# wdmwhh/MRefSR

Hardware: NVIDIA B200
Metric: x4 SR images/sec through the reference-alignment hot path (match + DCNv2 + fusion), 5 refs @160^2 HR (higher is better)
Workload: dtype f32 I/O (matcher: split-bf16 x3 operands on tcgen05, fp32 accumulate, diagonal form; dcn: tf32 operands, fp32 accumulate; fusion: fp32)

## Files before the change

include/mrefsr_b200.h:

```cpp
#ifndef MREFSR_B200_H_
#define MREFSR_B200_H_

#include <stddef.h>
#include <stdint.h>

#ifdef __cplusplus
extern "C" {
#endif

#define MREFSR_ABI_VERSION 1

#if defined(__GNUC__)
#define MREFSR_API __attribute__((visibility("default")))
#else
#define MREFSR_API
#endif

MREFSR_API int mrefsr_abi_version(void);
MREFSR_API const char* mrefsr_last_error(void);
MREFSR_API int mrefsr_sm_count(void);

enum {
    MREFSR_MATCH_AUTO = 0,
    MREFSR_MATCH_TC_BF16X3 = 1,
// ... 16 lines not shown
                                 void* stream);

MREFSR_API int mrefsr_pre_offsets(const int64_t* max_idx, int n, int h, int w, float* out_s1, float* out_s2, float* out_s4,
                       void* stream);

enum {
    MREFSR_DCN_AUTO = 0,
    MREFSR_DCN_FP32 = 1,
    MREFSR_DCN_TF32 = 2,
    MREFSR_DCN_TF32X3 = 3,
};
MREFSR_API size_t mrefsr_dcn_workspace_bytes(int B, int C, int H, int W, int Co, int kh, int kw, int stride_h, int stride_w,
                                  int pad_h, int pad_w, int dil_h, int dil_w, int group, int deformable_group,
                                  int mode, int backward);
MREFSR_API int mrefsr_dcn_tile_plan(int B, int Ho, int Wo, int* meta, int* coords, size_t max_rows);
MREFSR_API int mrefsr_modulated_deform_conv_forward(const float* input, const float* weight, const float* bias,
                                         const float* offset, const float* mask, float* output, int B, int C, int H,
                                         int W, int Co, int kh, int kw, int stride_h, int stride_w, int pad_h,
                                         int pad_w, int dil_h, int dil_w, int group, int deformable_group,
                                         int with_bias, int mode, void* workspace, size_t workspace_bytes,
                                         void* stream);
MREFSR_API int mrefsr_modulated_deform_conv_backward(const float* input, const float* weight, const float* offset,
                                          const float* mask, const float* grad_output, float* grad_input,
                                          float* grad_weight, float* grad_bias, float* grad_offset, float* grad_mask,
                                          int B, int C, int H, int W, int Co, int kh, int kw, int stride_h,
                                          int stride_w, int pad_h, int pad_w, int dil_h, int dil_w, int group,
                                          int deformable_group, int with_bias, int mode, void* workspace,
                                          size_t workspace_bytes, void* stream);

MREFSR_API int mrefsr_dynagg_offsets(const float* conv_out, const float* pre_offset, float* offset, float* mask,
// ... 118 lines not shown
```

mrefsr_b200/_lib.py:

```python
import ctypes
import os
import threading

import torch

_HERE = os.path.dirname(os.path.abspath(__file__))
LIB_PATH = os.environ.get('MREFSR_LIB') or os.path.join(_HERE, 'lib', 'libmrefsr_b200.so')

c_int, c_size_t, c_void_p = ctypes.c_int, ctypes.c_size_t, ctypes.c_void_p

_I = c_int
_P = c_void_p
SIGNATURES = {
    'mrefsr_abi_version': (c_int, []),
    'mrefsr_last_error': (ctypes.c_char_p, []),
    'mrefsr_sm_count': (c_int, []),
    'mrefsr_match_workspace_bytes': (c_size_t, [_I] * 8),
    'mrefsr_match_plan': (c_int, [_I] * 9 + [_P]),
    'mrefsr_feature_match_batched': (c_int, [_P, _P] + [_I] * 15 + [_P, _P, _P, c_size_t, _P]),
    'mrefsr_pre_offsets': (c_int, [_P, _I, _I, _I, _P, _P, _P, _P]),
    'mrefsr_dcn_workspace_bytes': (c_size_t, [_I] * 17),
    'mrefsr_dcn_tile_plan': (c_int, [_I, _I, _I, _P, _P, c_size_t]),
    'mrefsr_modulated_deform_conv_forward': (c_int, [_P] * 6 + [_I] * 17 + [_P, c_size_t, _P]),
    'mrefsr_modulated_deform_conv_backward': (c_int, [_P] * 10 + [_I] * 17 + [_P, c_size_t, _P]),
    'mrefsr_gemm_tf32_nt': (c_int, [_P, _I, ctypes.c_longlong, _P, _I, ctypes.c_longlong, _P, _I, ctypes.c_longlong,
                                    _I, _I, _I, _I, _I, _I, _P]),
    'mrefsr_gemm_tf32x3_nt': (c_int, [_P, _P, _I, ctypes.c_longlong, _P, _P, _I, ctypes.c_longlong, _P, _I,
                                      ctypes.c_longlong, _I, _I, _I, _I, _I, _I, _P]),
    'mrefsr_dcn_pack_weights': (c_int, [_P, _P, _I, _I, _I, _P]),
    'mrefsr_dcn_pack_weights_x3': (c_int, [_P, _P, _I, _I, _I, _P]),
    'mrefsr_dynagg_dcn_forward': (c_int, [_P] * 5 + [_I] + [_P] + [_I] * 7 + [_P, c_size_t, _P]),
    'mrefsr_dynagg_dcn_forward_multi': (c_int, [_P] * 5 + [_I] + [_P] + [_I] * 12 + [ctypes.c_float, _P, c_size_t, _P]),
    'mrefsr_dynagg_dcn_forward_slabs': (c_int, [_P] * 5 + [_I] + [_P] + [_I] * 13 + [ctypes.c_float, _P, c_size_t, _P]),
    'mrefsr_dynagg_dcn_forward_ex': (c_int, [_P] * 5 + [_I] + [_P] + [_I] * 8 + [ctypes.c_float, _P, c_size_t, _P]),
    'mrefsr_dynagg_dcn_backward': (c_int, [_P] * 4 + [_I] + [_P] * 5 + [_I] * 9 + [_P, c_size_t, _P]),
    'mrefsr_dynagg_offsets': (c_int, [_P] * 5 + [_I] * 5 + [_P]),
    'mrefsr_dynagg_offsets_backward': (c_int, [_P] * 4 + [_I] * 5 + [_P]),
# ... 101 lines not shown
```

mrefsr_b200/csrc/dcn.cu:

```cuda
#include <type_traits>

#include "common.cuh"
#include "dcn_tc.cuh"
#include "../../include/mrefsr_b200.h"

namespace mrefsr {

constexpr int DT = 64;
constexpr int DK = 16;

__global__ void __launch_bounds__(256)
dcn_fwd_simt_kernel(const float* __restrict__ x, const float* __restrict__ offset, const float* __restrict__ mask,
                    const float* __restrict__ weight, const float* __restrict__ bias, float* __restrict__ out,
                    const DcnShape s) {
    __shared__ float As[DK][DT + 4];
    __shared__ float Bs[DK][DT + 4];
    const int K = s.kh * s.kw, P = s.Ho * s.Wo, cpg = s.C / s.G, opg = s.Co / s.G, cdg = s.C / s.DG;
    const int oct = cdiv_d(opg, DT);
    const int b = blockIdx.z, gi = blockIdx.y / oct, ot = blockIdx.y % oct;
    const int p0 = blockIdx.x * DT, oc0 = ot * DT;
    const int t = threadIdx.x;
    const int lpos = t & 63, lkq = (t >> 6) * 4;
    const int ty = t >> 4, tx = t & 15;
    const int p = p0 + lpos;
// ... 956 lines not shown
    return 0;
}

}

using namespace mrefsr;

extern "C" {

int mrefsr_dcn_tile_plan(int B, int Ho, int Wo, int* meta, int* coords, size_t max_rows) {
    MREFSR_CHECK(B > 0 && Ho > 0 && Wo > 0 && meta, ERR_BAD_ARG, "tile plan: bad arguments");
    MREFSR_CHECK((long long)B * Ho * Wo < (1ll << 31) - 256, ERR_BAD_ARG, "tile plan: too many positions");
    return dcn_tc_tile_plan(B, Ho, Wo, meta, coords, max_rows);
}

size_t mrefsr_dcn_workspace_bytes(int B, int C, int H, int W, int Co, int kh, int kw, int stride_h, int stride_w,
                                  int pad_h, int pad_w, int dil_h, int dil_w, int group, int deformable_group, int mode,
                                  int backward) {
    DcnShape s;
    if (dcn_make_shape(&s, B, C, H, W, Co, kh, kw, stride_h, stride_w, pad_h, pad_w, dil_h, dil_w, group,
                       deformable_group))
        return 0;
    if (backward) {
        const bool x3 = mode == MREFSR_DCN_TF32X3;
        const size_t buf = align_up((size_t)bwd_chunk(s, x3) * C * kh * kw * s.Ho * s.Wo * 4, 1024);
        const size_t got = align_up((size_t)B * Co * s.Ho * s.Wo * 4, 1024), gwt = align_up((size_t)Co * C * kh * kw * 4, 1024);
        return 2 * buf + align_up((size_t)B * C * H * W * 4, 1024) + 2 * got + 2 * gwt +
               align_up((size_t)BWD_MAX_SPLITS * Co * C * kh * kw * 4, 1024) + (x3 ? buf + 2 * got + gwt : 0) + 1024;
    }
    return dcn_tc_workspace_bytes(s, mode) + 1024;
// ... 279 lines not shown
```

mrefsr_b200/csrc/dcn_common.cuh:

```cuda
#pragma once
#include "common.cuh"

namespace mrefsr {

struct DcnShape {
    int B, C, H, W, Co, kh, kw, sh, sw, ph, pw, dh, dw, G, DG, Ho, Wo;
};

__host__ __device__ __forceinline__ int cdiv_d(int a, int b) { return (a + b - 1) / b; }

struct PlaneSrc {};
struct DynAggSrc {
    const long long* max_idx;
    int flow_scale, hp, wp, x_nhwc;
};

#ifdef __CUDACC__
__device__ __forceinline__ float dcn_sample(const float* __restrict__ plane, int H, int W, float y, float x) {
    if (!(y > -1.f && x > -1.f && y < (float)H && x < (float)W)) return 0.f;
    const int y0 = (int)floorf(y), x0 = (int)floorf(x);
    const int y1 = y0 + 1, x1 = x0 + 1;
    const float ly = y - (float)y0, lx = x - (float)x0, hy = 1.f - ly, hx = 1.f - lx;
    const float a = (y0 >= 0 && x0 >= 0) ? __ldg(plane + y0 * W + x0) : 0.f;
    const float b = (y0 >= 0 && x1 <= W - 1) ? __ldg(plane + y0 * W + x1) : 0.f;
// ... 19 lines not shown
int dcn_pack_weights(const float* w, float* wt, int Co, int C, int K, cudaStream_t st, bool x3 = false);

struct DcnOutputs {
    float* ptr[8];
    int n, group, stride, offset;
    int slab_rows;
};

bool dcn_tc_eligible(const DcnShape& s);
size_t dcn_tc_workspace_bytes(const DcnShape& s, int mode);
int dcn_forward_tc_impl(const float* x, const float* w, const float* bias, const float* off, const float* mask,
                        const long long* max_idx, int flow_scale, float* out, const DcnShape& s, void* workspace,
                        size_t workspace_bytes, cudaStream_t st, int layout_flags, float out_slope,
                        const DcnOutputs* multi);
int dcn_tc_tile_plan(int B, int Ho, int Wo, int* meta, int* coords, size_t max_rows);
int dcn_forward_tc(const float* x, const float* w, const float* bias, const float* off, const float* mask, float* out,
                   const DcnShape& s, void* workspace, size_t workspace_bytes, cudaStream_t st, bool x3);

}
```

mrefsr_b200/csrc/dcn_tc.cu:

```cuda
#include <stdlib.h>
#include "dcn_tc.cuh"
#include "../../include/mrefsr_b200.h"

namespace mrefsr {


template <bool ROUND,
          bool SPLIT = false>
__global__ void __launch_bounds__(256)
nchw_to_nhwc_kernel(const float* __restrict__ src, float* __restrict__ dst, int C, int HW, float* __restrict__ dst_lo) {
    __shared__ float tile[128][33];
    const int b = blockIdx.z, p0 = blockIdx.x * 32, c0 = blockIdx.y * 128;
    const int lane = threadIdx.x & 31, warp = threadIdx.x >> 5;
    const float* s = src + (size_t)b * C * HW;
    float* d = dst + (size_t)b * C * HW;
    const int p = p0 + lane;
#pragma unroll
    for (int i = 0; i < 16; ++i) {
        const int cl = warp + 8 * i, c = c0 + cl;
        const float v = (c < C && p < HW) ? __ldcs(s + (size_t)c * HW + p) : 0.f;
        tile[cl][lane] = (ROUND && !SPLIT) ? to_tf32(v) : v;
    }
    __syncthreads();
#pragma unroll
// ... 23 lines not shown
}

__global__ void dcn_weight_repack_x3_kernel(const float* __restrict__ w, float* __restrict__ wt, int Co, int C, int K) {
    const int total = Co * C * K;
    for (int i = blockIdx.x * blockDim.x + threadIdx.x; i < total; i += gridDim.x * blockDim.x) {
        const int c = i % C, tap = (i / C) % K, co = i / (C * K);
        const float v = __ldg(w + ((size_t)co * C + c) * K + tap), hi = to_tf32(v);
        float* o = wt + ((size_t)co * K + tap) * 2 * C + (c / TBK_X3) * 2 * TBK_X3 + c % TBK_X3;
        o[0] = hi;
        o[TBK_X3] = to_tf32(v - hi);
    }
}


__device__ __forceinline__ void dcn_epilogue_tile(const DcnTcParams& prm, const float* __restrict__ bias,
                                                  uint32_t tmem_base, uint64_t* tempty_bar, int tile, int buf, int warp,
                                                  int lane, int half_lo, int half_hi) {
    const int Co = prm.s.Co, P = prm.P;
#pragma unroll 1
    for (int half = half_lo; half < half_hi; ++half) {
        int b = 0, oy = 0, ox = 0;
        const bool ok = dcn_row_coords(prm, tile, half * 128 + warp * 32 + lane, b, oy, ox);
        const int p = ok ? oy * prm.s.Wo + ox : 0;
        if (!ok) b = 0;
        const int bd = prm.dst_group ? (b / prm.dst_group) * prm.dst_stride + prm.dst_offset + b % prm.dst_group : b;
        int k_lo = 0, k_hi = prm.n_outs, Pd = P;
        size_t o_off = prm.out_nhwc ? ((size_t)bd * P + p) * Co : (size_t)bd * Co * P + p;
        if (prm.dst_slab_rows) {
            k_lo = oy / prm.dst_slab_rows;
            k_hi = k_lo + 1;
            Pd = prm.dst_slab_rows * prm.s.Wo;
            o_off = (size_t)bd * Co * Pd + (size_t)(oy - k_lo * prm.dst_slab_rows) * prm.s.Wo + ox;
        }
        const uint32_t taddr = tmem_base + ((uint32_t)(warp * 32) << 16) + buf * 2 * Co + half * Co;
#pragma unroll 1
        for (int c0 = 0; c0 < Co; c0 += 8) {
            uint32_t v[8];
            tmem_ld_32x8(taddr + c0, v);
            tmem_ld_wait();
#ifdef MREFSR_DCN_DEBUG
            if (prm.dbg & 16) continue;
#endif
            if (ok) {
                float f[8];
#pragma unroll
                for (int e = 0; e < 8; ++e) {
                    f[e] = __uint_as_float(v[e]) + (bias ? __ldg(bias + c0 + e) : 0.f);
                    f[e] = f[e] > 0.f ? f[e] : f[e] * prm.out_slope;
                }
#pragma unroll 1
                for (int k = k_lo; k < k_hi; ++k) {
                    float* o = prm.outs[k] + o_off;
                    if (prm.out_nhwc) {
                        *reinterpret_cast<float4*>(o + c0) = make_float4(f[0], f[1], f[2], f[3]);
                        *reinterpret_cast<float4*>(o + c0 + 4) = make_float4(f[4], f[5], f[6], f[7]);
                    } else {
#pragma unroll
                        for (int e = 0; e < 8; ++e) o[(size_t)(c0 + e) * Pd] = f[e];
                    }
                }
            }
        }
    }
    tc_fence_before();
    __syncwarp();
    if (lane == 0) mbar_arrive(tempty_bar);
}

template <bool X3>
__device__ __forceinline__ void dcn_mma_issuer(const DcnTcParams& prm, uint8_t* smem, uint64_t* full, uint64_t* empty,
                                               uint64_t* tfull, uint64_t* tempty, uint32_t tmem_base, int nkb_tile) {
    const int Co = prm.s.Co, S = prm.stages;
    const uint32_t idesc = umma_idesc(2, 128, Co);
    int stage = 0, it = 0;
    uint32_t phase = 0;
    for (int tile = blockIdx.x; tile < prm.tiles; tile += gridDim.x, ++it) {
        const int buf = it & (prm.nbuf - 1);
        const uint32_t bphase = (it >> (prm.nbuf - 1)) & 1;
        mbar_wait_backoff(&tempty[buf], bphase ^ 1, 32);
        tc_fence_after();
        const uint32_t tacc = tmem_base + buf * 2 * Co;
        uint32_t accumulate = 0;
        for (int kb = 0; kb < nkb_tile; ++kb) {
            mbar_wait_backoff(&full[stage], phase, 20);
            tc_fence_after();
            const uint32_t sa = smem_u32(smem + (size_t)stage * prm.stage_bytes);
            const uint32_t sb = sa + T_A_BYTES;
            if (X3) {
#pragma unroll
                for (int kk = 0; kk < 2; ++kk) {
#ifdef MREFSR_DCN_DEBUG
                    if (prm.dbg & 8) continue;
#endif
                    const uint64_t bh = umma_desc_sw128(sb + kk * 32, 0), bl = umma_desc_sw128(sb + (kk + 2) * 32, 0);
#pragma unroll
                    for (int half = 0; half < 2; ++half) {
                        const uint32_t ah = sa + half * (128 * 128) + kk * 32;
                        umma_tf32(tacc + half * Co, umma_desc_sw128(ah + 64, 0), bh, idesc, accumulate);
// ... 11 lines not shown
                    const uint64_t db = umma_desc_sw128(sb + kk * 32, 0);
                    umma_tf32(tacc, umma_desc_sw128(sa + kk * 32, 0), db, idesc, accumulate);
                    umma_tf32(tacc + Co, umma_desc_sw128(sa + 128 * 128 + kk * 32, 0), db, idesc, accumulate);
                    accumulate = 1;
                }
            }
            umma_commit(&empty[stage]);
            if (++stage == S) {
                stage = 0;
                phase ^= 1;
            }
        }
        umma_commit(&tfull[buf]);
    }
}

constexpr int S_GW = 16;
constexpr int S_DW = 8;
constexpr int S_MMA_WARP = S_GW + S_DW;
constexpr int S_THREADS = (S_GW + S_DW + 1) * 32;
#ifndef MREFSR_S_NTAB
#define MREFSR_S_NTAB 4
#endif
constexpr int S_NTAB = MREFSR_S_NTAB;
static_assert((S_NTAB & (S_NTAB - 1)) == 0, "ring slot and phase are derived from the K-step index");

template <int GS>
struct DcnRaw {
    float dy[GS], dx[GS], mk[GS];
    int mi, fyx;
};

template <bool FUSED, int GS,
          bool X3 = false>
__global__ void __launch_bounds__(S_THREADS, 1)
dcn_tc_split_kernel(const __grid_constant__ CUtensorMap mapW, const float* __restrict__ xt,
                    const float* __restrict__ offset, const float* __restrict__ mask,
                    const long long* __restrict__ max_idx, const float* __restrict__ bias,
                    const __grid_constant__ DcnTcParams prm) {
    extern __shared__ __align__(1024) uint8_t smem[];
    if ((smem_u32(smem) & 1023u) != 0u) __trap();
    const DcnShape& s = prm.s;
    const int S = prm.stages;
    uint64_t* bars = reinterpret_cast<uint64_t*>(smem + (size_t)S * prm.stage_bytes);
    uint64_t* full = bars;
    uint64_t* empty = bars + S;
    uint64_t* tfull = bars + 2 * S;
    uint64_t* tempty = tfull + 2;
    uint64_t* tab_full = tempty + 2;
    uint64_t* tab_empty = tab_full + S_NTAB;
    uint32_t* tmem_slot = reinterpret_cast<uint32_t*>(tab_empty + S_NTAB);
    constexpr int tab_n = GS * TAB_STRIDE;
    int* tab_base = reinterpret_cast<int*>(reinterpret_cast<uint8_t*>(bars) + 256);
    float* tab_w = reinterpret_cast<float*>(tab_base + S_NTAB * tab_n);

    const int warp = threadIdx.x >> 5, lane = threadIdx.x & 31;
// ... 9 lines not shown
        for (int a = 0; a < 2; ++a) {
            mbar_init(&tfull[a], 1);
            mbar_init(&tempty[a], 8);
        }
        for (int a = 0; a < S_NTAB; ++a) {
            mbar_init(&tab_full[a], S_DW);
            mbar_init(&tab_empty[a], S_GW / 2);
        }
        fence_mbar_init();
    }
    if (warp == S_MMA_WARP) tmem_alloc<512>(tmem_slot);
    tc_fence_before();
    __syncthreads();
    tc_fence_after();
    const uint32_t tmem_base = *tmem_slot;
    const int my_tiles = (prm.tiles - (int)blockIdx.x + (int)gridDim.x - 1) / (int)gridDim.x;
    const int total_kb = my_tiles * nkb_tile;

    if (warp < S_GW) {
        constexpr int SLAB = X3 ? TBK_X3 : TBK;
        constexpr int ITEMS = X3 ? 2 : 4;
        constexpr int RSTEP = TBM / ITEMS;
        const int grp = warp >> 3;
        const int tg = threadIdx.x & 255;
        const int ch = tg & (SLAB / 8 - 1);
        const int r0 = tg >> (X3 ? 1 : 2);
        const int gsub = (ch * 8) / prm.cdg;
        const uint32_t a_off0 = (uint32_t)r0 * 128u + (uint32_t)(((2 * ch) ^ (r0 & 7)) << 4);
        const uint32_t a_off1 = (uint32_t)r0 * 128u + (uint32_t)(((2 * ch + 1) ^ (r0 & 7)) << 4);
        const uint32_t a_off2 = (uint32_t)r0 * 128u + (uint32_t)(((2 * ch + 4) ^ (r0 & 7)) << 4);
        const uint32_t a_off3 = (uint32_t)r0 * 128u + (uint32_t)(((2 * ch + 5) ^ (r0 & 7)) << 4);
        const bool is_epi = (warp & 7) < 4;
        int ep_done = 0, prod_done = 0;
        const int nbuf_mask = prm.nbuf - 1;
        auto poll_epilogue = [&]() {
            if (is_epi && ep_done < prod_done) {
                const int buf = ep_done & nbuf_mask;
                if (mbar_try_wait(&tfull[buf], (ep_done >> nbuf_mask) & 1)) {
                    tc_fence_after();
                    dcn_epilogue_tile(prm, bias, tmem_base, &tempty[buf], (int)blockIdx.x + ep_done * (int)gridDim.x, buf,
                                      warp & 3, lane, grp, grp + 1);
                    ++ep_done;
                }
            }
        };
        auto wait_poll = [&](uint64_t* bar, uint32_t parity) {
            while (!mbar_try_wait(bar, parity)) poll_epilogue();
        };
        int stage = grp % S, c_slab = 0, c_tap = grp;
        uint32_t phase = 0;
        while (c_tap >= K) {
            c_tap -= K;
            if (++c_slab == prm.n_slabs) {
                c_slab = 0;
                ++prod_done;
            }
        }
        const int dx_elems = C, dy_elems = s.W * C;
        for (int kb = grp; kb < total_kb; kb += 2) {
            const int g_slot = kb & (S_NTAB - 1);
            const uint32_t g_phase = (uint32_t)(kb / S_NTAB) & 1u;
            poll_epilogue();
            const float* xs = xt + (c_slab * SLAB + ch * 8);
            const int* tb = tab_base + g_slot * tab_n + gsub * TAB_STRIDE + r0;
            const float* tw = tab_w + g_slot * 4 * tab_n + gsub * TAB_STRIDE + r0;
            wait_poll(&tab_full[g_slot], g_phase);
            wait_poll(&empty[stage], phase ^ 1);
            uint8_t* A = smem + (size_t)stage * prm.stage_bytes;
            if (tg == 0) {
                mbar_expect_tx(&full[stage], Co * 128);
                tma_load_3d(A + T_A_BYTES, &mapW, &full[stage], c_tap * (X3 ? 2 * C : C) + c_slab * TBK, 0, 0);
            }
// ... 40 lines not shown
            __syncwarp();
            if (lane == 0) {
                mbar_arrive(&full[stage]);
                mbar_arrive(&tab_empty[g_slot]);
            }
            stage += 2;
            if (stage >= S) {
                stage -= S;
                phase ^= 1;
            }
            c_tap += 2;
            while (c_tap >= K) {
                c_tap -= K;
                if (++c_slab == prm.n_slabs) {
                    c_slab = 0;
                    ++prod_done;
                }
            }
        }
        prod_done = my_tiles;
        while (is_epi && ep_done < prod_done) {
            const int buf = ep_done & nbuf_mask;
            mbar_wait_backoff(&tfull[buf], (ep_done >> nbuf_mask) & 1, 64);
            tc_fence_after();
            dcn_epilogue_tile(prm, bias, tmem_base, &tempty[buf], (int)blockIdx.x + ep_done * (int)gridDim.x, buf, warp & 3,
                              lane, grp, grp + 1);
            ++ep_done;
        }
    } else if (warp < S_MMA_WARP) {
        const int erow = threadIdx.x - S_GW * 32;
        int l_tile = blockIdx.x, l_slab = 0, l_tap = 0, l_dg0 = 0;
        const unsigned kw_magic = 65536u / (unsigned)s.kw + 1u;
        int row_yx = -1, row_bH = 0, row_qyx = 0, row_idx0 = 0;
        const float* row_off = offset;
        const float* row_msk = mask;
        auto decode_rows = [&](int tile) {
            int b = 0, oy = 0, ox = 0;
            row_yx = -1;
            if (dcn_row_coords(prm, tile, erow, b, oy, ox)) {
                const int p = oy * s.Wo + ox;
                row_yx = (oy << 16) | ox;
                row_bH = b * s.H;
                if (FUSED) {
                    row_off = offset + (size_t)b * 3 * s.DG * K * P + p;
                    row_qyx = ((oy / prm.flow_scale) << 16) | (ox / prm.flow_scale);
                    row_idx0 = b * prm.hp * prm.wp;
                } else {
                    row_off = offset + (size_t)b * 2 * s.DG * K * P + p;
                    if (mask) row_msk = mask + (size_t)b * s.DG * K * P + p;
                }
            }
        };
        struct RawRow {
            DcnRaw<GS> r;
            int yx, bH;
        };
        auto load_next = [&](RawRow& rr, int l_kb) {
            rr.yx = row_yx;
            rr.bH = row_bH;
            rr.r.fyx = -1;
#ifdef MREFSR_DCN_DEBUG
            if (row_yx >= 0 && !(prm.dbg & 2)) {
#else
            if (row_yx >= 0) {
#endif
#pragma unroll
                for (int g = 0; g < GS; ++g) {
                    {
                        const int dgi = l_dg0 + g;
                        if (!FUSED) {
                            const unsigned o = (unsigned)((dgi * 2 * K + 2 * l_tap) * P);
// ... 9 lines not shown
                    }
                }
                if (FUSED) {
                    const int l_ti = (int)(((unsigned)l_tap * kw_magic) >> 16), l_tj = l_tap - l_ti * s.kw;
                    const int fy = (row_qyx >> 16) - l_ti, fx = (row_qyx & 0xffff) - l_tj;
                    if (fy >= 0 && fx >= 0 && fy < prm.hp && fx < prm.wp) {
                        rr.r.mi = ldg_early_s32(reinterpret_cast<const int*>(max_idx + (row_idx0 + fy * prm.wp + fx)));
                        rr.r.fyx = (fy << 16) | fx;
                    }
                }
            }
            if (++l_tap == K) {
                l_tap = 0;
                if (++l_slab == prm.n_slabs) {
                    l_slab = 0;
                    l_tile += gridDim.x;
                    if (l_kb + 1 < total_kb) decode_rows(l_tile);
                }
                constexpr int SLAB = X3 ? TBK_X3 : TBK;
                l_dg0 = (prm.cdg >= SLAB) ? (l_slab * SLAB) / prm.cdg : l_slab * (SLAB / prm.cdg);
            }
        };
        int d_tap = 0;
        auto decode_store = [&](const RawRow& rr, int d_kb) {
            const int d_slot = d_kb & (S_NTAB - 1);
            const uint32_t d_phase = (uint32_t)(d_kb / S_NTAB) & 1u;
            mbar_wait(&tab_empty[d_slot], d_phase ^ 1);
            int* tb = tab_base + d_slot * tab_n + erow;
            float* tw = tab_w + d_slot * 4 * tab_n + erow;
            float ybase = 0.f, xbase = 0.f, fly = 0.f, flx = 0.f;
            if (rr.yx >= 0) {
                const int d_ti = (int)(((unsigned)d_tap * kw_magic) >> 16), d_tj = d_tap - d_ti * s.kw;
                ybase = (float)((rr.yx >> 16) * s.sh - s.ph + d_ti * s.dh);
                xbase = (float)((rr.yx & 0xffff) * s.sw - s.pw + d_tj * s.dw);
                if (FUSED && rr.r.fyx >= 0) {
                    const int my = (int)__umulhi((unsigned)rr.r.mi, prm.wp_magic), mx = rr.r.mi - my * prm.wp;
                    fly = (float)((my - (rr.r.fyx >> 16)) * prm.flow_scale);
                    flx = (float)((mx - (rr.r.fyx & 0xffff)) * prm.flow_scale);
// ... 33 lines not shown
                        w1 = (ty0 && tx1) ? w1 : 0.f;
                        w2 = (ty1 && tx0) ? w2 : 0.f;
                        w3 = (ty1 && tx1) ? w3 : 0.f;
                    }
                    const int e = g * TAB_STRIDE;
                    tb[e] = in ? base : 0;
                    tw[e] = in ? w0 : 0.f;
                    tw[e + tab_n] = in ? w1 : 0.f;
                    tw[e + 2 * tab_n] = in ? w2 : 0.f;
                    tw[e + 3 * tab_n] = in ? w3 : 0.f;
                }
            }
            __syncwarp();
            if (lane == 0) mbar_arrive(&tab_full[d_slot]);
            if (++d_tap == K) d_tap = 0;
        };
        RawRow ra, rb;
        ra.yx = rb.yx = -1;
        ra.bH = rb.bH = 0;
        ra.r.mi = rb.r.mi = 0;
        ra.r.fyx = rb.r.fyx = -1;
#pragma unroll
        for (int g = 0; g < GS; ++g) ra.r.dy[g] = ra.r.dx[g] = ra.r.mk[g] = rb.r.dy[g] = rb.r.dx[g] = rb.r.mk[g] = 0.f;
        if (total_kb > 0) {
            decode_rows(l_tile);
            load_next(ra, 0);
        }
        if (total_kb > 1) load_next(rb, 1);
        for (int kb = 0; kb < total_kb; kb += 2) {
            decode_store(ra, kb);
            if (kb + 2 < total_kb) load_next(ra, kb + 2);
            if (kb + 1 < total_kb) {
                decode_store(rb, kb + 1);
                if (kb + 3 < total_kb) load_next(rb, kb + 3);
            }
        }
    } else {
        if (lane == 0) dcn_mma_issuer<X3>(prm, smem, full, empty, tfull, tempty, tmem_base, nkb_tile);
        __syncwarp();
    }
    tc_fence_before();
    __syncthreads();
    if (warp == S_MMA_WARP) {
        tc_fence_after();
        tmem_dealloc<512>(tmem_base);
    }
}

int dcn_pack_weights(const float* w, float* wt, int Co, int C, int K, cudaStream_t st, bool x3) {
    if (x3) {
        MREFSR_CHECK(C % TBK_X3 == 0, ERR_BAD_ARG, "pack_weights (x3): C %% 16 != 0 (C = %d)", C);
        dcn_weight_repack_x3_kernel<<<cdiv(Co * C * K, 256), 256, 0, st>>>(w, wt, Co, C, K);
    } else {
        dcn_weight_repack_kernel<<<cdiv(Co * C * K, 256), 256, 0, st>>>(w, wt, Co, C, K);
    }
    MREFSR_LAUNCH_CHECK();
    count_launches(1);
    return 0;
}

int dcn_nchw_to_nhwc(const float* x, float* xt, int B, int C, int HW, cudaStream_t st, bool round_tf32, float* xt_lo) {
// ... 1 lines not shown
    if (xt_lo) nchw_to_nhwc_kernel<true, true><<<grid, 256, 0, st>>>(x, xt, C, HW, xt_lo);
    else if (round_tf32) nchw_to_nhwc_kernel<true><<<grid, 256, 0, st>>>(x, xt, C, HW, nullptr);
    else nchw_to_nhwc_kernel<false><<<grid, 256, 0, st>>>(x, xt, C, HW, nullptr);
    MREFSR_LAUNCH_CHECK();
    count_launches(1);
    return 0;
}

bool dcn_tc_eligible(const DcnShape& s) {
    const int cdg = s.C / s.DG;
    const bool slab_ok = (cdg >= TBK) ? (cdg % TBK == 0) : (TBK % cdg == 0 && cdg % 8 == 0);
    return s.G == 1 && s.C % TBK == 0 && slab_ok && s.Co % 32 == 0 && s.Co >= 32 && s.Co <= 256 &&
           (size_t)s.B * s.C * s.H * s.W < ((size_t)1 << 31) && s.Ho < 32768 && s.Wo < 65536;
}

size_t dcn_tc_workspace_bytes(const DcnShape& s, int mode) {
    if (mode == MREFSR_DCN_FP32 || !dcn_tc_eligible(s)) return 0;
    const size_t wfloats = (size_t)s.Co * s.C * s.kh * s.kw * (mode == MREFSR_DCN_TF32X3 ? 2 : 1);
    return align_up((size_t)s.B * s.C * s.H * s.W * 4, 1024) + align_up(wfloats * 4, 1024);
}

static void dcn_plan_tiles(DcnTcParams& prm) {
    const DcnShape& s = prm.s;
    prm.tiles = cdiv(prm.total_rows, TBM);
    prm.tile2d = prm.tx_log = prm.ty_log = prm.sub_log = prm.subs_log = prm.nsx = prm.nsub = 0;
    static const int cand[5][2] = {{4, 4}, {4, 3}, {3, 4}, {3, 3}, {5, 3}};
    long long best = -1;
    for (int k = 0; k < 5; ++k) {
        const int tx = cand[k][0], ty = cand[k][1];
        const long long nsx = cdiv(s.Wo, 1 << tx), nsy = cdiv(s.Ho, 1 << ty);
        const long long rows = (long long)s.B * nsx * nsy << (tx + ty);
        const long long tiles = (rows + TBM - 1) / TBM;
        if (best < 0 || tiles * 100 < best * 97) {
            best = tiles;
// ... 28 lines not shown
        MREFSR_CHECK((size_t)prm.tiles * TBM <= max_rows, ERR_BAD_ARG, "tile plan: %d rows, room for %zu", prm.tiles * TBM,
                     max_rows);
        for (int t = 0; t < prm.tiles; ++t)
            for (int r = 0; r < TBM; ++r) {
                int b = -1, oy = -1, ox = -1;
                if (!dcn_row_coords(prm, t, r, b, oy, ox)) b = oy = ox = -1;
                int* c = coords + ((size_t)t * TBM + r) * 3;
                c[0] = b;
                c[1] = oy;
                c[2] = ox;
            }
    }
    return 0;
}

static int make_weight_map(CUtensorMap* map, const float* wt, int Co, int Ktot) {
    return make_tensor_map_3d(map, CU_TENSOR_MAP_DATA_TYPE_FLOAT32, 4, wt, (uint64_t)Ktot, (uint64_t)Co, 1, TBK,
                              (uint32_t)Co, CU_TENSOR_MAP_SWIZZLE_128B);
}

int dcn_forward_tc_impl(const float* x, const float* w, const float* bias, const float* off, const float* mask,
                        const long long* max_idx, int flow_scale, float* out, const DcnShape& s, void* workspace,
                        size_t workspace_bytes, cudaStream_t st, int layout_flags, float out_slope,
                        const DcnOutputs* multi) {
    const bool x3 = (layout_flags & MREFSR_DCN_X3) != 0;
    const size_t need = dcn_tc_workspace_bytes(s, x3 ? MREFSR_DCN_TF32X3 : MREFSR_DCN_TF32);
    MREFSR_CHECK(workspace && workspace_bytes >= need, ERR_WORKSPACE, "dcn forward: workspace too small (%zu < %zu)",
                 workspace_bytes, need);
    MREFSR_CHECK((reinterpret_cast<uintptr_t>(workspace) & 1023) == 0, ERR_WORKSPACE,
                 "dcn forward: workspace must be 1024-byte aligned");
// ... 73 lines not shown

    prm.flow_scale = flow_scale;
    prm.hp = prm.wp = 0;
    prm.wp_magic = 0;
    if (prm.fused) {
        MREFSR_CHECK(flow_scale >= 1 && s.Ho % flow_scale == 0 && s.Wo % flow_scale == 0, ERR_BAD_ARG,
                     "fused DynAgg: output %dx%d not a multiple of the flow scale %d", s.Ho, s.Wo, flow_scale);
        prm.hp = s.Ho / flow_scale - 2;
        prm.wp = s.Wo / flow_scale - 2;
        MREFSR_CHECK(prm.hp > 0 && prm.wp > 1, ERR_BAD_ARG, "fused DynAgg: feature grid too small");
        MREFSR_CHECK((unsigned long long)prm.hp * prm.wp * prm.wp < (1ull << 32), ERR_BAD_ARG,
                     "fused DynAgg: feature grid %dx%d too large", prm.hp, prm.wp);
        prm.wp_magic = 0xFFFFFFFFu / (unsigned)prm.wp + 1u;
    }
    const size_t smem = (size_t)prm.stages * prm.stage_bytes + 256 + table_bytes + 1024;
    int grid = sm_count();
    if (grid > prm.tiles) grid = prm.tiles;
    using Kernel = decltype(&dcn_tc_split_kernel<false, 1>);
    static const Kernel kernels[2][3] = {
        {dcn_tc_split_kernel<false, 1>, dcn_tc_split_kernel<false, 2>, dcn_tc_split_kernel<false, 4>},
        {dcn_tc_split_kernel<true, 1>, dcn_tc_split_kernel<true, 2>, dcn_tc_split_kernel<true, 4>}};
    static const Kernel kernels_x3[2][2] = {
        {dcn_tc_split_kernel<false, 1, true>, dcn_tc_split_kernel<false, 2, true>},
        {dcn_tc_split_kernel<true, 1, true>, dcn_tc_split_kernel<true, 2, true>}};
    const Kernel kern = x3 ? kernels_x3[prm.fused][prm.gs >> 1] : kernels[prm.fused][prm.gs >> 1];
    ScopedTiming tm(MREFSR_K_DCN_FWD, st);
    MREFSR_CUDA(cudaFuncSetAttribute(kern, cudaFuncAttributeMaxDynamicSharedMemorySize, (int)smem));
    kern<<<grid, S_THREADS, smem, st>>>(mapW, xt, off, prm.fused ? nullptr : mask, prm.fused ? max_idx : nullptr, bias,
                                        prm);
    MREFSR_LAUNCH_CHECK();
    count_launches(1);
    return 0;
}

int dcn_forward_tc(const float* x, const float* w, const float* bias, const float* off, const float* mask, float* out,
                   const DcnShape& s, void* workspace, size_t workspace_bytes, cudaStream_t st, bool x3) {
    return dcn_forward_tc_impl(x, w, bias, off, mask, nullptr, 1, out, s, workspace, workspace_bytes, st,
                               x3 ? MREFSR_DCN_X3 : 0, 1.f, nullptr);
}

}
```

mrefsr_b200/csrc/dcn_tc.cuh:

```cuda
#pragma once
#include "dcn_common.cuh"

namespace mrefsr {

constexpr int TBM = 256;
constexpr int TBK = 32;
constexpr int TBK_X3 = 16;
constexpr int T_A_BYTES = TBM * 128;
constexpr int T_SMEM_BUDGET = 150 * 1024;

struct DcnTcParams {
    DcnShape s;
    int P, total_rows, tiles, n_slabs, taps, cdg, gs, stages, nbuf, stage_bytes;
    int fused, flow_scale, hp, wp;
    float* outs[8];
    int n_outs, dst_group, dst_stride, dst_offset;
    int dst_slab_rows;
    int out_nhwc;
    float out_slope;
    unsigned wp_magic;
    int tile2d, tx_log, ty_log, sub_log, subs_log, nsx, nsub;
    int dbg;
};

__host__ __device__ __forceinline__ bool dcn_row_coords(const DcnTcParams& prm, int tile, int r, int& b, int& oy, int& ox) {
    if (!prm.tile2d) {
        const int m = tile * TBM + r;
        if (m >= prm.total_rows) return false;
        b = m / prm.P;
        const int p = m - b * prm.P;
        oy = p / prm.s.Wo;
        ox = p - oy * prm.s.Wo;
        return true;
    }
    const int st = (tile << prm.subs_log) + (r >> prm.sub_log);
    const int within = r & ((1 << prm.sub_log) - 1);
    b = st / prm.nsub;
    const int rem = st - b * prm.nsub, ty = rem / prm.nsx, tx = rem - ty * prm.nsx;
// ... 27 lines not shown
}

struct F8 {
    float2 v[4];
};
__device__ __forceinline__ F8 ldg8(const float* p) {
    F8 r;
    asm("ld.global.nc.v8.f32 {%0,%1,%2,%3,%4,%5,%6,%7}, [%8];"
        : "=f"(r.v[0].x), "=f"(r.v[0].y), "=f"(r.v[1].x), "=f"(r.v[1].y), "=f"(r.v[2].x), "=f"(r.v[2].y),
          "=f"(r.v[3].x), "=f"(r.v[3].y)
        : "l"(p));
    return r;
}
constexpr int TAB_STRIDE = TBM + 4;

__device__ __forceinline__ int ldg_early_s32(const int* p) {
    int v;
    asm volatile("ld.global.nc.s32 %0, [%1];" : "=r"(v) : "l"(p));
    return v;
}

}
```

Measured before the change: 3205.

## Add stream-K tail scheduling to the persistent tcgen05 DCN kernel

Replaces the plain round-robin tile loop in the persistent DCN tensor-core kernel with a hybrid data-parallel plus stream-K schedule. When the last wave would leave at least a tenth of the CTAs idle, the remaining tiles' K-steps are split evenly across CTAs. Partial accumulators are combined through a global scratch buffer with atomic arrival counters and acquire/release flags. This targets wave-quantization tail idle time, at the cost of extra workspace, a memset per launch, spin-waits between CTAs and more complex producer/loader seek logic.

```diff
diff --git a/include/mrefsr_b200.h b/include/mrefsr_b200.h
--- a/include/mrefsr_b200.h
+++ b/include/mrefsr_b200.h
@@ -54,6 +54,7 @@
                                   int pad_h, int pad_w, int dil_h, int dil_w, int group, int deformable_group,
                                   int mode, int backward);
 MREFSR_API int mrefsr_dcn_tile_plan(int B, int Ho, int Wo, int* meta, int* coords, size_t max_rows);
+MREFSR_API int mrefsr_dcn_work_plan(int tiles, int sms, int nkb_tile, int* counts, int* units, size_t max_units);
 MREFSR_API int mrefsr_modulated_deform_conv_forward(const float* input, const float* weight, const float* bias,
                                          const float* offset, const float* mask, float* output, int B, int C, int H,
                                          int W, int Co, int kh, int kw, int stride_h, int stride_w, int pad_h,
diff --git a/mrefsr_b200/_lib.py b/mrefsr_b200/_lib.py
--- a/mrefsr_b200/_lib.py
+++ b/mrefsr_b200/_lib.py
@@ -21,6 +21,7 @@
     'mrefsr_pre_offsets': (c_int, [_P, _I, _I, _I, _P, _P, _P, _P]),
     'mrefsr_dcn_workspace_bytes': (c_size_t, [_I] * 17),
     'mrefsr_dcn_tile_plan': (c_int, [_I, _I, _I, _P, _P, c_size_t]),
+    'mrefsr_dcn_work_plan': (c_int, [_I, _I, _I, _P, _P, c_size_t]),
     'mrefsr_modulated_deform_conv_forward': (c_int, [_P] * 6 + [_I] * 17 + [_P, c_size_t, _P]),
     'mrefsr_modulated_deform_conv_backward': (c_int, [_P] * 10 + [_I] * 17 + [_P, c_size_t, _P]),
     'mrefsr_gemm_tf32_nt': (c_int, [_P, _I, ctypes.c_longlong, _P, _I, ctypes.c_longlong, _P, _I, ctypes.c_longlong,
diff --git a/mrefsr_b200/csrc/dcn.cu b/mrefsr_b200/csrc/dcn.cu
--- a/mrefsr_b200/csrc/dcn.cu
+++ b/mrefsr_b200/csrc/dcn.cu
@@ -994,6 +994,12 @@
     return dcn_tc_tile_plan(B, Ho, Wo, meta, coords, max_rows);
 }
 
+int mrefsr_dcn_work_plan(int tiles, int sms, int nkb_tile, int* counts, int* units, size_t max_units) {
+    MREFSR_CHECK(tiles > 0 && sms > 0 && nkb_tile > 0 && counts, ERR_BAD_ARG, "work plan: bad arguments");
+    MREFSR_CHECK((long long)2 * sms * nkb_tile < (1ll << 31), ERR_BAD_ARG, "work plan: too many K steps");
+    return dcn_tc_work_plan(tiles, sms, nkb_tile, counts, units, max_units);
+}
+
 size_t mrefsr_dcn_workspace_bytes(int B, int C, int H, int W, int Co, int kh, int kw, int stride_h, int stride_w,
                                   int pad_h, int pad_w, int dil_h, int dil_w, int group, int deformable_group, int mode,
                                   int backward) {
diff --git a/mrefsr_b200/csrc/dcn_common.cuh b/mrefsr_b200/csrc/dcn_common.cuh
--- a/mrefsr_b200/csrc/dcn_common.cuh
+++ b/mrefsr_b200/csrc/dcn_common.cuh
@@ -57,6 +57,7 @@
                         size_t workspace_bytes, cudaStream_t st, int layout_flags, float out_slope,
                         const DcnOutputs* multi);
 int dcn_tc_tile_plan(int B, int Ho, int Wo, int* meta, int* coords, size_t max_rows);
+int dcn_tc_work_plan(int tiles, int sms, int nkb, int* counts, int* units, size_t max_units);
 int dcn_forward_tc(const float* x, const float* w, const float* bias, const float* off, const float* mask, float* out,
                    const DcnShape& s, void* workspace, size_t workspace_bytes, cudaStream_t st, bool x3);
 
diff --git a/mrefsr_b200/csrc/dcn_tc.cu b/mrefsr_b200/csrc/dcn_tc.cu
--- a/mrefsr_b200/csrc/dcn_tc.cu
+++ b/mrefsr_b200/csrc/dcn_tc.cu
@@ -61,11 +61,24 @@
 
 
 __device__ __forceinline__ void dcn_epilogue_tile(const DcnTcParams& prm, const float* __restrict__ bias,
-                                                  uint32_t tmem_base, uint64_t* tempty_bar, int tile, int buf, int warp,
-                                                  int lane, int half_lo, int half_hi) {
+                                                  uint32_t tmem_base, uint64_t* tempty_bar, int tile, int split, int buf,
+                                                  int warp, int lane, int half_lo, int half_hi) {
     const int Co = prm.s.Co, P = prm.P;
 #pragma unroll 1
     for (int half = half_lo; half < half_hi; ++half) {
+        float* part = nullptr;
+        unsigned* ready = nullptr;
+        bool first = false;
+        if (split >= 0) {
+            const int q = (split * 2 + half) * 4 + warp;
+            unsigned old = 0;
+            if (lane == 0) old = atomicAdd(prm.sk_flags + q, 1u);
+            first = __shfl_sync(0xffffffffu, old, 0) == 0u;
+            ready = prm.sk_flags + prm.sk_slots * 8 + q;
+            part = prm.sk_part + (size_t)q * 32 * Co + lane * 8;
+            if (!first)
+                while (ld_acquire_gpu(ready) == 0u) __nanosleep(64);
+        }
         int b = 0, oy = 0, ox = 0;
         const bool ok = dcn_row_coords(prm, tile, half * 128 + warp * 32 + lane, b, oy, ox);
         const int p = ok ? oy * prm.s.Wo + ox : 0;
@@ -85,6 +98,25 @@
             uint32_t v[8];
             tmem_ld_32x8(taddr + c0, v);
             tmem_ld_wait();
+            if (part) {
+                float4* pp = reinterpret_cast<float4*>(part + c0 * 32);
+                if (first) {
+                    __stcg(pp, make_float4(__uint_as_float(v[0]), __uint_as_float(v[1]), __uint_as_float(v[2]),
+                                           __uint_as_float(v[3])));
+                    __stcg(pp + 1, make_float4(__uint_as_float(v[4]), __uint_as_float(v[5]), __uint_as_float(v[6]),
+                                               __uint_as_float(v[7])));
+                    continue;
+                }
+                const float4 a = __ldcg(pp), b = __ldcg(pp + 1);
+                v[0] = __float_as_uint(__uint_as_float(v[0]) + a.x);
+                v[1] = __float_as_uint(__uint_as_float(v[1]) + a.y);
+                v[2] = __float_as_uint(__uint_as_float(v[2]) + a.z);
+                v[3] = __float_as_uint(__uint_as_float(v[3]) + a.w);
+                v[4] = __float_as_uint(__uint_as_float(v[4]) + b.x);
+                v[5] = __float_as_uint(__uint_as_float(v[5]) + b.y);
+                v[6] = __float_as_uint(__uint_as_float(v[6]) + b.z);
+                v[7] = __float_as_uint(__uint_as_float(v[7]) + b.w);
+            }
 #ifdef MREFSR_DCN_DEBUG
             if (prm.dbg & 16) continue;
 #endif
@@ -108,6 +140,11 @@
                 }
             }
         }
+        if (first) {
+            __threadfence();
+            __syncwarp();
+            if (lane == 0) st_release_gpu(ready, 1u);
+        }
     }
     tc_fence_before();
     __syncwarp();
@@ -119,16 +156,18 @@
                                                uint64_t* tfull, uint64_t* tempty, uint32_t tmem_base, int nkb_tile) {
     const int Co = prm.s.Co, S = prm.stages;
     const uint32_t idesc = umma_idesc(2, 128, Co);
-    int stage = 0, it = 0;
+    const DcnCtaSched w = dcn_cta_sched(prm.dp_rounds, prm.dp_full, prm.sk_kb, gridDim.x, nkb_tile, blockIdx.x);
+    int stage = 0;
     uint32_t phase = 0;
-    for (int tile = blockIdx.x; tile < prm.tiles; tile += gridDim.x, ++it) {
+    for (int it = 0; it < w.n_units; ++it) {
+        const DcnWorkUnit wu = dcn_work_unit(w, gridDim.x, nkb_tile, blockIdx.x, it);
         const int buf = it & (prm.nbuf - 1);
         const uint32_t bphase = (it >> (prm.nbuf - 1)) & 1;
         mbar_wait_backoff(&tempty[buf], bphase ^ 1, 32);
         tc_fence_after();
         const uint32_t tacc = tmem_base + buf * 2 * Co;
         uint32_t accumulate = 0;
-        for (int kb = 0; kb < nkb_tile; ++kb) {
+        for (int kb = wu.kb_begin; kb < wu.kb_end; ++kb) {
             mbar_wait_backoff(&full[stage], phase, 20);
             tc_fence_after();
             const uint32_t sa = smem_u32(smem + (size_t)stage * prm.stage_bytes);
@@ -170,6 +209,14 @@
         umma_commit(&tfull[buf]);
     }
 }
+
+#ifdef MREFSR_DCN_DEBUG
+__device__ __forceinline__ unsigned long long globaltimer_ns() {
+    unsigned long long t;
+    asm volatile("mov.u64 %0, %globaltimer;" : "=l"(t));
+    return t;
+}
+#endif
 
 constexpr int S_GW = 16;
 constexpr int S_DW = 8;
@@ -196,6 +243,9 @@
                     const __grid_constant__ DcnTcParams prm) {
     extern __shared__ __align__(1024) uint8_t smem[];
     if ((smem_u32(smem) & 1023u) != 0u) __trap();
+#ifdef MREFSR_DCN_DEBUG
+    if (prm.dbg_clock && threadIdx.x == 0) prm.dbg_clock[2 * blockIdx.x] = globaltimer_ns();
+#endif
     const DcnShape& s = prm.s;
     const int S = prm.stages;
     uint64_t* bars = reinterpret_cast<uint64_t*>(smem + (size_t)S * prm.stage_bytes);
@@ -235,8 +285,8 @@
     __syncthreads();
     tc_fence_after();
     const uint32_t tmem_base = *tmem_slot;
-    const int my_tiles = (prm.tiles - (int)blockIdx.x + (int)gridDim.x - 1) / (int)gridDim.x;
-    const int total_kb = my_tiles * nkb_tile;
+    const DcnCtaSched sched = dcn_cta_sched(prm.dp_rounds, prm.dp_full, prm.sk_kb, gridDim.x, nkb_tile, blockIdx.x);
+    const int total_kb = sched.total_kb;
 
     if (warp < S_GW) {
         constexpr int SLAB = X3 ? TBK_X3 : TBK;
@@ -259,8 +309,9 @@
                 const int buf = ep_done & nbuf_mask;
                 if (mbar_try_wait(&tfull[buf], (ep_done >> nbuf_mask) & 1)) {
                     tc_fence_after();
-                    dcn_epilogue_tile(prm, bias, tmem_base, &tempty[buf], (int)blockIdx.x + ep_done * (int)gridDim.x, buf,
-                                      warp & 3, lane, grp, grp + 1);
+                    const DcnWorkUnit wu = dcn_work_unit(sched, gridDim.x, nkb_tile, blockIdx.x, ep_done);
+                    dcn_epilogue_tile(prm, bias, tmem_base, &tempty[buf], wu.tile,
+                                      dcn_split_slot(wu, nkb_tile, blockIdx.x), buf, warp & 3, lane, grp, grp + 1);
                     ++ep_done;
                 }
             }
@@ -268,15 +319,14 @@
         auto wait_poll = [&](uint64_t* bar, uint32_t parity) {
             while (!mbar_try_wait(bar, parity)) poll_epilogue();
         };
-        int stage = grp % S, c_slab = 0, c_tap = grp;
+        int stage = grp % S, c_slab = 0, c_tap = 0;
         uint32_t phase = 0;
-        while (c_tap >= K) {
-            c_tap -= K;
-            if (++c_slab == prm.n_slabs) {
-                c_slab = 0;
-                ++prod_done;
-            }
-        }
+        auto locate = [&](int kb) {
+            dcn_locate_kb(sched, nkb_tile, kb, prod_done, c_tap);
+            c_slab = c_tap / K;
+            c_tap -= c_slab * K;
+        };
+        locate(grp);
         const int dx_elems = C, dy_elems = s.W * C;
         for (int kb = grp; kb < total_kb; kb += 2) {
             const int g_slot = kb & (S_NTAB - 1);
@@ -347,22 +397,26 @@
                 c_tap -= K;
                 if (++c_slab == prm.n_slabs) {
                     c_slab = 0;
-                    ++prod_done;
-                }
-            }
-        }
-        prod_done = my_tiles;
+                    if (++prod_done == sched.n_dp) {
+                        locate(kb + 2);
+                        break;
+                    }
+                }
+            }
+        }
+        prod_done = sched.n_units;
         while (is_epi && ep_done < prod_done) {
             const int buf = ep_done & nbuf_mask;
             mbar_wait_backoff(&tfull[buf], (ep_done >> nbuf_mask) & 1, 64);
             tc_fence_after();
-            dcn_epilogue_tile(prm, bias, tmem_base, &tempty[buf], (int)blockIdx.x + ep_done * (int)gridDim.x, buf, warp & 3,
-                              lane, grp, grp + 1);
+            const DcnWorkUnit wu = dcn_work_unit(sched, gridDim.x, nkb_tile, blockIdx.x, ep_done);
+            dcn_epilogue_tile(prm, bias, tmem_base, &tempty[buf], wu.tile, dcn_split_slot(wu, nkb_tile, blockIdx.x), buf,
+                              warp & 3, lane, grp, grp + 1);
             ++ep_done;
         }
     } else if (warp < S_MMA_WARP) {
         const int erow = threadIdx.x - S_GW * 32;
-        int l_tile = blockIdx.x, l_slab = 0, l_tap = 0, l_dg0 = 0;
+        int l_tile = 0, l_slab = 0, l_tap = 0, l_dg0 = 0;
         const unsigned kw_magic = 65536u / (unsigned)s.kw + 1u;
         int row_yx = -1, row_bH = 0, row_qyx = 0, row_idx0 = 0;
         const float* row_off = offset;
@@ -388,6 +442,16 @@
             DcnRaw<GS> r;
             int yx, bH;
         };
+        constexpr int SLAB = X3 ? TBK_X3 : TBK;
+        auto seek = [&](int l_kb) {
+            int u = 0;
+            dcn_locate_kb(sched, nkb_tile, l_kb, u, l_tap);
+            l_tile = dcn_work_unit(sched, gridDim.x, nkb_tile, blockIdx.x, u).tile;
+            l_slab = l_tap / K;
+            l_tap -= l_slab * K;
+            l_dg0 = (prm.cdg >= SLAB) ? (l_slab * SLAB) / prm.cdg : l_slab * (SLAB / prm.cdg);
+            decode_rows(l_tile);
+        };
         auto load_next = [&](RawRow& rr, int l_kb) {
             rr.yx = row_yx;
             rr.bH = row_bH;
@@ -427,14 +491,22 @@
                 l_tap = 0;
                 if (++l_slab == prm.n_slabs) {
                     l_slab = 0;
-                    l_tile += gridDim.x;
-                    if (l_kb + 1 < total_kb) decode_rows(l_tile);
-                }
-                constexpr int SLAB = X3 ? TBK_X3 : TBK;
+                    if (l_kb + 1 < total_kb) {
+                        if (l_tile + (int)gridDim.x < sched.sk_tile0) {
+                            l_tile += gridDim.x;
+                            decode_rows(l_tile);
+                        } else if (l_tile >= sched.sk_tile0) {
+                            decode_rows(++l_tile);
+                        } else {
+                            seek(l_kb + 1);
+                            return;
+                        }
+                    }
+                }
                 l_dg0 = (prm.cdg >= SLAB) ? (l_slab * SLAB) / prm.cdg : l_slab * (SLAB / prm.cdg);
             }
         };
-        int d_tap = 0;
+        int d_tap = (sched.n_dp ? 0 : sched.g0 % nkb_tile) % K;
         auto decode_store = [&](const RawRow& rr, int d_kb) {
             const int d_slot = d_kb & (S_NTAB - 1);
             const uint32_t d_phase = (uint32_t)(d_kb / S_NTAB) & 1u;
@@ -498,6 +570,7 @@
             __syncwarp();
             if (lane == 0) mbar_arrive(&tab_full[d_slot]);
             if (++d_tap == K) d_tap = 0;
+            if (d_kb + 1 == prm.dp_rounds * nkb_tile) d_tap = (sched.g0 % nkb_tile) % K;
         };
         RawRow ra, rb;
         ra.yx = rb.yx = -1;
@@ -507,7 +580,7 @@
 #pragma unroll
         for (int g = 0; g < GS; ++g) ra.r.dy[g] = ra.r.dx[g] = ra.r.mk[g] = rb.r.dy[g] = rb.r.dx[g] = rb.r.mk[g] = 0.f;
         if (total_kb > 0) {
-            decode_rows(l_tile);
+            seek(0);
             load_next(ra, 0);
         }
         if (total_kb > 1) load_next(rb, 1);
@@ -529,6 +602,9 @@
         tc_fence_after();
         tmem_dealloc<512>(tmem_base);
     }
+#ifdef MREFSR_DCN_DEBUG
+    if (prm.dbg_clock && threadIdx.x == 0) prm.dbg_clock[2 * blockIdx.x + 1] = globaltimer_ns();
+#endif
 }
 
 int dcn_pack_weights(const float* w, float* wt, int Co, int C, int K, cudaStream_t st, bool x3) {
@@ -560,10 +636,29 @@
            (size_t)s.B * s.C * s.H * s.W < ((size_t)1 << 31) && s.Ho < 32768 && s.Wo < 65536;
 }
 
+static void dcn_plan_tiles(DcnTcParams& prm);
+static void dcn_schedule(int tiles, int sms, int nkb, int& grid, int& dp_rounds, int& dp_full, int& sk_kb);
+
+static int dcn_split_slots(const DcnShape& s) {
+    DcnTcParams prm;
+    memset(&prm, 0, sizeof(prm));
+    prm.s = s;
+    prm.P = s.Ho * s.Wo;
+    prm.total_rows = s.B * prm.P;
+    dcn_plan_tiles(prm);
+    const int sms = sm_count();
+    if (sms <= 0) return 0;
+    int grid = 0, dp_rounds = 0, dp_full = 0, sk_kb = 0;
+    dcn_schedule(prm.tiles, sms, 1, grid, dp_rounds, dp_full, sk_kb);
+    return sk_kb ? grid : 0;
+}
+
 size_t dcn_tc_workspace_bytes(const DcnShape& s, int mode) {
     if (mode == MREFSR_DCN_FP32 || !dcn_tc_eligible(s)) return 0;
     const size_t wfloats = (size_t)s.Co * s.C * s.kh * s.kw * (mode == MREFSR_DCN_TF32X3 ? 2 : 1);
-    return align_up((size_t)s.B * s.C * s.H * s.W * 4, 1024) + align_up(wfloats * 4, 1024);
+    const size_t slots = dcn_split_slots(s);
+    return align_up((size_t)s.B * s.C * s.H * s.W * 4, 1024) + align_up(wfloats * 4, 1024) +
+           (slots ? align_up(slots * 16 * 4, 1024) + slots * TBM * s.Co * 4 : 0);
 }
 
 static void dcn_plan_tiles(DcnTcParams& prm) {
@@ -622,6 +717,39 @@
     return 0;
 }
 
+static void dcn_schedule(int tiles, int sms, int nkb, int& grid, int& dp_rounds, int& dp_full, int& sk_kb) {
+    grid = sms < tiles ? sms : tiles;
+    dp_rounds = (tiles + grid - 1) / grid;
+    dp_full = tiles - (dp_rounds - 1) * grid;
+    sk_kb = 0;
+    if ((long long)(dp_rounds * grid - tiles) * 10 >= (long long)dp_rounds * grid) {
+        dp_rounds = tiles / grid - 1;
+        dp_full = grid;
+        sk_kb = (tiles - dp_rounds * grid) * nkb;
+    }
+}
+
+int dcn_tc_work_plan(int tiles, int sms, int nkb, int* counts, int* units, size_t max_units) {
+    int grid = 0, dp_rounds = 0, dp_full = 0, sk_kb = 0;
+    dcn_schedule(tiles, sms, nkb, grid, dp_rounds, dp_full, sk_kb);
+    size_t n = 0;
+    for (int cta = 0; cta < sms; ++cta) {
+        counts[cta] = 0;
+        if (cta >= grid) continue;
+        const DcnCtaSched w = dcn_cta_sched(dp_rounds, dp_full, sk_kb, grid, nkb, cta);
+        counts[cta] = w.n_units;
+        if (!units) continue;
+        MREFSR_CHECK(n + w.n_units <= max_units, ERR_BAD_ARG, "work plan: room for %zu units", max_units);
+        for (int u = 0; u < w.n_units; ++u, ++n) {
+            const DcnWorkUnit r = dcn_work_unit(w, grid, nkb, cta, u);
+            units[3 * n] = r.tile;
+            units[3 * n + 1] = r.kb_begin;
+            units[3 * n + 2] = r.kb_end;
+        }
+    }
+    return 0;
+}
+
 static int make_weight_map(CUtensorMap* map, const float* wt, int Co, int Ktot) {
     return make_tensor_map_3d(map, CU_TENSOR_MAP_DATA_TYPE_FLOAT32, 4, wt, (uint64_t)Ktot, (uint64_t)Co, 1, TBK,
                               (uint32_t)Co, CU_TENSOR_MAP_SWIZZLE_128B);
@@ -725,8 +853,14 @@
         prm.wp_magic = 0xFFFFFFFFu / (unsigned)prm.wp + 1u;
     }
     const size_t smem = (size_t)prm.stages * prm.stage_bytes + 256 + table_bytes + 1024;
-    int grid = sm_count();
-    if (grid > prm.tiles) grid = prm.tiles;
+    int grid = 0;
+    dcn_schedule(prm.tiles, sm_count(), prm.n_slabs * K, grid, prm.dp_rounds, prm.dp_full, prm.sk_kb);
+    prm.sk_slots = prm.sk_kb ? grid : 0;
+    uint8_t* sk_ws = static_cast<uint8_t*>(workspace) + align_up((size_t)s.B * s.C * s.H * s.W * 4, 1024) +
+                     align_up((size_t)s.Co * s.C * K * (x3 ? 2 : 1) * 4, 1024);
+    prm.sk_flags = reinterpret_cast<unsigned*>(sk_ws);
+    prm.sk_part = reinterpret_cast<float*>(sk_ws + align_up((size_t)prm.sk_slots * 16 * 4, 1024));
+    prm.dbg_clock = nullptr;
     using Kernel = decltype(&dcn_tc_split_kernel<false, 1>);
     static const Kernel kernels[2][3] = {
         {dcn_tc_split_kernel<false, 1>, dcn_tc_split_kernel<false, 2>, dcn_tc_split_kernel<false, 4>},
@@ -736,11 +870,33 @@
         {dcn_tc_split_kernel<true, 1, true>, dcn_tc_split_kernel<true, 2, true>}};
     const Kernel kern = x3 ? kernels_x3[prm.fused][prm.gs >> 1] : kernels[prm.fused][prm.gs >> 1];
     ScopedTiming tm(MREFSR_K_DCN_FWD, st);
+    if (prm.sk_slots) MREFSR_CUDA(cudaMemsetAsync(prm.sk_flags, 0, (size_t)prm.sk_slots * 16 * 4, st));
     MREFSR_CUDA(cudaFuncSetAttribute(kern, cudaFuncAttributeMaxDynamicSharedMemorySize, (int)smem));
+#ifdef MREFSR_DCN_DEBUG
+    static unsigned long long* clk = nullptr;
+    const char* clk_path = getenv("MREFSR_DCN_CLOCK");
+    if (clk_path && !clk) MREFSR_CUDA(cudaMalloc(&clk, 2 * 1024 * sizeof(unsigned long long)));
+    if (clk_path && grid <= 1024) prm.dbg_clock = clk;
+#endif
     kern<<<grid, S_THREADS, smem, st>>>(mapW, xt, off, prm.fused ? nullptr : mask, prm.fused ? max_idx : nullptr, bias,
                                         prm);
     MREFSR_LAUNCH_CHECK();
     count_launches(1);
+#ifdef MREFSR_DCN_DEBUG
+    if (prm.dbg_clock) {
+        unsigned long long h[2 * 1024];
+        MREFSR_CUDA(cudaMemcpyAsync(h, clk, 2 * grid * sizeof(unsigned long long), cudaMemcpyDeviceToHost, st));
+        MREFSR_CUDA(cudaStreamSynchronize(st));
+        FILE* f = fopen(clk_path, "a");
+        if (f) {
+            fprintf(f, "{\"C\": %d, \"Co\": %d, \"H\": %d, \"tiles\": %d, \"grid\": %d, \"x3\": %d, \"t\": [", s.C, s.Co,
+                    s.H, prm.tiles, grid, x3 ? 1 : 0);
+            for (int i = 0; i < 2 * grid; ++i) fprintf(f, i ? ", %llu" : "%llu", h[i]);
+            fprintf(f, "]}\n");
+            fclose(f);
+        }
+    }
+#endif
     return 0;
 }
 
diff --git a/mrefsr_b200/csrc/dcn_tc.cuh b/mrefsr_b200/csrc/dcn_tc.cuh
--- a/mrefsr_b200/csrc/dcn_tc.cuh
+++ b/mrefsr_b200/csrc/dcn_tc.cuh
@@ -20,8 +20,60 @@
     float out_slope;
     unsigned wp_magic;
     int tile2d, tx_log, ty_log, sub_log, subs_log, nsx, nsub;
+    int dp_rounds, dp_full, sk_kb;
+    float* sk_part;
+    unsigned* sk_flags;
+    int sk_slots;
     int dbg;
+    unsigned long long* dbg_clock;
 };
+
+struct DcnWorkUnit {
+    int tile, kb_begin, kb_end;
+};
+struct DcnCtaSched {
+    int n_dp, sk_tile0, g0, g1;
+    int n_units, total_kb;
+};
+__host__ __device__ __forceinline__ DcnCtaSched dcn_cta_sched(int dp_rounds, int dp_full, int sk_kb, int grid, int nkb,
+                                                              int cta) {
+    DcnCtaSched w;
+    w.n_dp = dp_rounds;
+    w.sk_tile0 = dp_rounds * grid;
+    w.g0 = (int)((long long)cta * sk_kb / grid);
+    w.g1 = (int)((long long)(cta + 1) * sk_kb / grid);
+    const int n_rr = dp_rounds - (cta >= dp_full ? 1 : 0);
+    w.n_units = n_rr + (w.g1 + nkb - 1) / nkb - w.g0 / nkb;
+    w.total_kb = n_rr * nkb + w.g1 - w.g0;
+    return w;
+}
+__host__ __device__ __forceinline__ DcnWorkUnit dcn_work_unit(const DcnCtaSched& w, int grid, int nkb, int cta, int u) {
+    DcnWorkUnit r;
+    if (u < w.n_dp) {
+        r.tile = cta + u * grid;
+        r.kb_begin = 0;
+        r.kb_end = nkb;
+    } else {
+        const int j = w.g0 / nkb + u - w.n_dp;
+        r.tile = w.sk_tile0 + j;
+        r.kb_begin = w.g0 > j * nkb ? w.g0 - j * nkb : 0;
+        r.kb_end = w.g1 - j * nkb < nkb ? w.g1 - j * nkb : nkb;
+    }
+    return r;
+}
+__host__ __device__ __forceinline__ void dcn_locate_kb(const DcnCtaSched& w, int nkb, int kb, int& u, int& k) {
+    if (kb < w.n_dp * nkb) {
+        u = kb / nkb;
+        k = kb - u * nkb;
+    } else {
+        const int g = w.g0 + kb - w.n_dp * nkb, j = g / nkb;
+        u = w.n_dp + j - w.g0 / nkb;
+        k = g - j * nkb;
+    }
+}
+__host__ __device__ __forceinline__ int dcn_split_slot(const DcnWorkUnit& r, int nkb, int cta) {
+    return r.kb_end < nkb ? cta : (r.kb_begin > 0 ? cta - 1 : -1);
+}
 
 __host__ __device__ __forceinline__ bool dcn_row_coords(const DcnTcParams& prm, int tile, int r, int& b, int& oy, int& ox) {
     if (!prm.tile2d) {
@@ -79,6 +131,15 @@
 }
 constexpr int TAB_STRIDE = TBM + 4;
 
+__device__ __forceinline__ unsigned ld_acquire_gpu(const unsigned* p) {
+    unsigned v;
+    asm volatile("ld.acquire.gpu.global.u32 %0, [%1];" : "=r"(v) : "l"(p) : "memory");
+    return v;
+}
+__device__ __forceinline__ void st_release_gpu(unsigned* p, unsigned v) {
+    asm volatile("st.release.gpu.global.u32 [%0], %1;" :: "l"(p), "r"(v) : "memory");
+}
+
 __device__ __forceinline__ int ldg_early_s32(const int* p) {
     int v;
     asm volatile("ld.global.nc.s32 %0, [%1];" : "=r"(v) : "l"(p));
```

Measured after the change: 3214 (median of 6 runs). No clear change (+0.3%).
